# dek226/CSE375-FinalProj-Huffman-Decoding

Measured on AMD Instinct MI355X. Metric: decoded GB/s, higher is better.
Workload: dtype u8

## Files before the change

### cse375-finalproj-huffman-decoding_amd/csrc/gh_tile.hip

```cpp

#ifndef GH_TILE_TB
#define GH_TILE_TB 1024
#endif
constexpr int TILE_TB = GH_TILE_TB;
#ifndef GH_TILE_U
#define GH_TILE_U 3
#endif
constexpr int TILE_U = GH_TILE_U;
constexpr int TILE_U3 = 2;
constexpr int TILE_NS = 4;
constexpr int TILE_SCAP = 20;
constexpr int TILE_MIDG = 2;
constexpr int STAGE_PAD = 16;
#ifndef GH_TILE_LAG
#define GH_TILE_LAG 2
#endif
constexpr int TILE_LAG = GH_TILE_LAG;
constexpr int TILE_SLOTS = 16;
#ifndef GH_TILE_STAMPS
#define GH_TILE_STAMPS 0
#endif
#if GH_TILE_STAMPS
#define TSTAMP(i) (ts[i] = __builtin_amdgcn_s_memtime())
#else
#define TSTAMP(i) ((void)0)
#endif
#ifndef GH_TILE_CSUB
#define GH_TILE_CSUB 0
#endif
#ifndef GH_TILE_CLDS
#define GH_TILE_CLDS 0
#endif
#ifndef GH_TILE_LMAJ
#define GH_TILE_LMAJ 1
#endif
#ifndef GH_TILE_POLLDIV
#define GH_TILE_POLLDIV 1
#endif
#ifndef GH_TILE_DYN
#define GH_TILE_DYN 0
#endif
constexpr int TILE_TAHEAD = 5;
#ifndef GH_TILE_LATEP
#define GH_TILE_LATEP 0
#endif
#ifndef GH_TILE_EPERM
#define GH_TILE_EPERM 0
#endif
#ifndef GH_TILE_HOLD
#define GH_TILE_HOLD 0
#endif
#ifndef GH_TILE_ALRD
#define GH_TILE_ALRD 1
#endif
#ifndef GH_TILE_W2
#define GH_TILE_W2 0
#endif
#ifndef GH_TILE_PF2
#define GH_TILE_PF2 0
#endif
#ifndef GH_TILE_ABLATE
#define GH_TILE_ABLATE 0
#endif
typedef unsigned int tile_v4u __attribute__((ext_vector_type(4)));
__device__ __forceinline__ void tile_st16(uint4* d, const uint4& v) {
  __builtin_nontemporal_store(tile_v4u{v.x, v.y, v.z, v.w}, (tile_v4u*)d);
}

struct TileParams {
  const uint32_t* payload;
  const uint32_t* gaps;
  const uint32_t* lut;
  uint8_t* out;
  unsigned long long* granules;
  unsigned long long* prefix;
  unsigned int* status;
  unsigned long long* total;
  unsigned long long* stats;
  unsigned long long out_cap;
  unsigned long long nseg;
  unsigned int gap_nib0, first_start, ntiles, kbits, lgr, epoch;
  unsigned int lut_bytes;
  unsigned int idle_block;
  unsigned int stage_bytes;
  unsigned int kbits_c;
  unsigned int fb_hi;
  unsigned int* tickets;
  uint4* stamps;
  unsigned long long* tstamps;
};

inline size_t tile_lds_bytes(size_t lut_bytes, size_t stage_bytes) {
  return lut_bytes + TILE_LAG * (TILE_TB / 64) * stage_bytes + TILE_SLOTS * (2 * (TILE_TB / 64) + 1) * 4 +
         TILE_SLOTS * 12 + 4 * (TILE_TB / 64) + 4 * TILE_SLOTS + 32;
}

__device__ __forceinline__ constexpr uint32_t perm_sel(int j) {
  return j == 0 ? 0x03020105u : j == 1 ? 0x03020500u : j == 2 ? 0x03050100u : 0x05020100u;
}

__device__ __forceinline__ void make_ewin(uint4 w, uint32_t w4, int start, uint32_t S, uint32_t (&e)[5]) {
  const uint32_t r = S - (uint32_t)start;
  e[0] = __builtin_amdgcn_alignbit(0u, w.x, r);
  e[1] = __builtin_amdgcn_alignbit(w.x, w.y, r);
  e[2] = __builtin_amdgcn_alignbit(w.y, w.z, r);
  e[3] = __builtin_amdgcn_alignbit(w.z, w.w, r);
  e[4] = __builtin_amdgcn_alignbit(w.w, w4, r);
}

constexpr uint32_t Q_SYMROOM = 0x7FFFu << 8;
constexpr uint32_t Q_LIVE = 128u << 23;
__device__ __forceinline__ uint32_t q_init(bool act, int start) {
  return ((act ? (uint32_t)(127 - start) : 511u) << 23) | Q_SYMROOM | 32u;
}

template <int N>
__device__ __forceinline__ void lds_wait_n(uint32_t& v) {
  static_assert(N >= 0 && N <= 3, "lgkmcnt 0..3");
  if constexpr (GH_TILE_CLDS) return;
  if constexpr (N == 0) asm volatile("s_waitcnt lgkmcnt(0)" : "+v"(v)::"memory");
  else if constexpr (N == 1) asm volatile("s_waitcnt lgkmcnt(1)" : "+v"(v)::"memory");
  else if constexpr (N == 2) asm volatile("s_waitcnt lgkmcnt(2)" : "+v"(v)::"memory");
  else asm volatile("s_waitcnt lgkmcnt(3)" : "+v"(v)::"memory");
}

template <int G, int U, int OW, int MINL, class Mid>
__device__ __forceinline__ int decode_tile_rolling(uint32_t (&e)[U][5], const int (&start)[U], const bool (&act)[U],
                                                   uint32_t (&ow)[U][OW], uint32_t (&cnt)[U], uint32_t amask,
                                                   uint32_t laneoff, Mid&& mid) {
  constexpr int S = 4 * OW;
  constexpr int NG = (S + G - 1) / G;
  constexpr int PLACE = GH_TILE_EPERM ? GH_TILE_EPERM : (G >= 4 ? 2 : 0);
  uint32_t q[U], ent[U];
#if GH_TILE_CLDS
  const __attribute__((address_space(3))) uint8_t* const lds0 = (const __attribute__((address_space(3))) uint8_t*)nullptr;
  auto lut_rd = [&](uint32_t a) -> uint32_t { return *(const __attribute__((address_space(3))) uint32_t*)(lds0 + a); };
#else
  auto lut_rd = [&](uint32_t a) -> uint32_t { return lds_u32_nowait(a); };
#endif
#pragma unroll
  for (int u = 0; u < U; ++u) {
    q[u] = q_init(act[u], start[u]);
    cnt[u] = 0;
#pragma unroll
    for (int k = 0; k < OW; ++k) asm volatile("" : "=v"(ow[u][k]));
  }
#pragma unroll
  for (int u = 0; u < U; ++u) ent[u] = lut_rd((e[u][0] & amask) | laneoff);
  int gdone = NG;
#pragma clang loop unroll(full)
  for (int gi = 0; gi < NG; ++gi) {
    const int CMIN = (gi + 1) * G * MINL;
    uint32_t qmin = 0xFFFFFFFFu;
#pragma clang loop unroll(full)
    for (int j = 0; j < G; ++j) {
      const int pos = gi * G + j;
      if (pos < S) {
        const bool gend = (j == G - 1) || (pos + 1 >= S);
        const bool last = gend && gi + 1 >= NG;
#pragma clang loop unroll(full)
        for (int u = 0; u < U; ++u) {
          if (last) {
            if constexpr (U == 3) {
              if (u == 0) lds_wait_n<2>(ent[u]);
              else if (u == 1) lds_wait_n<1>(ent[u]);
              else lds_wait_n<0>(ent[u]);
            } else if constexpr (U == 2) {
              if (u == 0) lds_wait_n<1>(ent[u]);
              else lds_wait_n<0>(ent[u]);
            } else {
              lds_wait_n<0>(ent[u]);
            }
          } else {
            lds_wait_n<U - 1>(ent[u]);
          }
#if GH_TILE_CSUB
          {
            uint32_t nq;
            const bool br = __builtin_sub_overflow(q[u], ent[u], &nq);
            q[u] = nq;
            cnt[u] = br ? (uint32_t)(pos + 1) : cnt[u];
          }
#else
          asm("v_sub_co_u32 %0, vcc, %0, %2\n\t"
              "v_cndmask_b32_e64 %1, %1, %3, vcc"
              : "+v"(q[u]), "+v"(cnt[u]) : "v"(ent[u]), "i"(pos + 1) : "vcc");
#endif
          ow[u][pos >> 2] = __builtin_amdgcn_perm(ent[u], ow[u][pos >> 2], perm_sel(pos & 3));
          if (PLACE == 1) asm volatile("" : "+v"(ow[u][pos >> 2]));
          if (!gend) {
            const uint32_t x = __builtin_amdgcn_alignbit(e[u][0], e[u][1], q[u]);
            ent[u] = lut_rd((x & amask) | laneoff);
          } else {
            e[u][0] = __builtin_amdgcn_alignbit(e[u][0], e[u][1], q[u]);
            if (CMIN + 32 < 157) e[u][1] = __builtin_amdgcn_alignbit(e[u][1], e[u][2], q[u]);
            if (CMIN + 64 < 157) e[u][2] = __builtin_amdgcn_alignbit(e[u][2], e[u][3], q[u]);
            if (CMIN + 96 < 157) e[u][3] = __builtin_amdgcn_alignbit(e[u][3], e[u][4], q[u]);
            if (CMIN + 128 < 157) e[u][4] = __builtin_amdgcn_alignbit(e[u][4], 0u, q[u]);
            q[u] = (q[u] & 0xFFFFFF00u) | 32u;
            qmin = min(qmin, q[u]);
            if (!last) ent[u] = lut_rd((e[u][0] & amask) | laneoff);
          }
        }
      }
    }
    if (PLACE == 2) {
#pragma unroll
      for (int u = 0; u < U; ++u) {
        const int w0 = (gi * G) >> 2, w1 = min(OW - 1, (gi * G + G - 1) >> 2);
#pragma unroll
        for (int wi = w0; wi <= w1; ++wi) asm volatile("" : "+v"(ow[u][wi]));
      }
    }
    if (gi == TILE_MIDG) mid();
    if (gi >= TILE_MIDG && gi + 1 < NG && !__any(qmin < Q_LIVE)) {
#pragma unroll
      for (int u = 0; u < U; ++u) lds_wait_n<0>(ent[u]);
      gdone = gi + 1;
      break;
    }
  }
  return gdone;
}

template <int OFF = 0>
__device__ __forceinline__ void lds_st32(uint32_t a, uint32_t v) {
  asm volatile("ds_write_b32 %0, %1 offset:%2" ::"v"(a), "v"(v), "i"(OFF) : "memory");
}
__device__ __forceinline__ uint32_t lds_ld_u32(uint32_t a) {
  uint32_t v;
  asm volatile("ds_read_b32 %0, %1\n\ts_waitcnt lgkmcnt(0)" : "=v"(v) : "v"(a) : "memory");
  return v;
}
__device__ __forceinline__ void lds_st_u32(uint32_t a, uint32_t v) {
  asm volatile("ds_write_b32 %0, %1\n\ts_waitcnt lgkmcnt(0)" ::"v"(a), "v"(v) : "memory");
}
__device__ __forceinline__ void lds_st32_m(uint32_t a, uint32_t v, int m) {
  switch (m) {
    case 1: lds_st32<4>(a, v); break;
    case 2: lds_st32<8>(a, v); break;
    case 3: lds_st32<12>(a, v); break;
    case 4: lds_st32<16>(a, v); break;
    case 5: lds_st32<20>(a, v); break;
    case 6: lds_st32<24>(a, v); break;
    case 7: lds_st32<28>(a, v); break;
    case 8: lds_st32<32>(a, v); break;
    case 9: lds_st32<36>(a, v); break;
    case 10: lds_st32<40>(a, v); break;
    case 11: lds_st32<44>(a, v); break;
    default: lds_st32<0>(a + 4u * (uint32_t)m, v); break;
  }
}
template <int U, int OW>
__device__ __forceinline__ void stage_wave(const uint32_t (&ow)[U][OW], const uint32_t (&n)[U], const uint32_t (&o)[U],
                                           int mmax) {
  uint32_t base[U], sh[U];
#pragma unroll
  for (int u = 0; u < U; ++u) {
    const uint32_t ap = ((o[u] - 1u) & 3u) + 1u;
    base[u] = o[u] - ap;
    sh[u] = 4u - ap;
  }
  auto dw = [&](int u, int m) { return __builtin_amdgcn_alignbyte(m < OW ? ow[u][m] : 0u, ow[u][m - 1], sh[u]); };
  if constexpr (GH_TILE_W2) {
#pragma unroll
    for (int m = OW; m >= 1; m -= 2) {
      if (m - 1 >= 1) {
        if (m <= mmax) {
#pragma unroll
          for (int u = 0; u < U; ++u)
            asm volatile("ds_write2_b32 %0, %1, %2 offset0:%3 offset1:%4" ::"v"(base[u]), "v"(dw(u, m)),
                         "v"(dw(u, m - 1)), "i"(m), "i"(m - 1) : "memory");
        } else if (m - 1 <= mmax) {
#pragma unroll
          for (int u = 0; u < U; ++u) lds_st32_m(base[u], dw(u, m - 1), m - 1);
        }
      } else if (m <= mmax) {
#pragma unroll
        for (int u = 0; u < U; ++u) lds_st32_m(base[u], dw(u, m), m);
      }
    }
  } else {
#pragma unroll
    for (int m = OW; m >= 1; --m) {
      if (m > mmax) continue;
#pragma unroll
      for (int u = 0; u < U; ++u) lds_st32_m(base[u], dw(u, m), m);
    }
  }
  uint32_t rd[U];
#pragma unroll
  for (int u = 0; u < U; ++u) rd[u] = lds_u32_nowait(base[u]);
  lds_wait(rd);
#pragma unroll
  for (int u = 0; u < U; ++u) {
    const uint32_t ap = o[u] - base[u];
    if (n[u] && ap < 4u) {
      const uint32_t ab = 8u * ap;
      lds_st32(base[u], (rd[u] & ((1u << ab) - 1u)) | (ow[u][0] << ab));
    }
  }
}

constexpr uint32_t OOB_OFF = 0x80000000u;
template <int NS, bool PIN = true>
__device__ __forceinline__ void copy_out_piece(uint8_t* out, uint32_t stg, unsigned long long goff, uint32_t n,
                                               int lane, tile_v4u (&v)[NS], uint32_t& b, uint32_t c0 = 0) {
  goff = rfl_u64(goff);
  n = (uint32_t)__builtin_amdgcn_readfirstlane((int)n);
  const uint32_t lb = (uint32_t)(goff & 15);
  const __amdgpu_buffer_rsrc_t rs = __builtin_amdgcn_make_buffer_rsrc(out + (goff - lb), 0, 0x7FFFFFF0, 0x00020000);
  const uint32_t src = (stg + 16u - ((GH_TILE_ABLATE & 128) ? 0u : lb)) & ((GH_TILE_ABLATE & 256) ? ~3u : ~0u);
  const uint32_t cf = lb ? 1u : 0u;
  const uint32_t ce = n ? (lb + n) >> 4 : 0u;
  uint32_t off[NS];
#pragma unroll
  for (int i = 0; i < NS; ++i) {
    const uint32_t c = c0 + cf + (uint32_t)lane + 64u * (uint32_t)i;
    off[i] = c < ce ? 16u * c : OOB_OFF;
  }
  const uint32_t nh = (lb && n) ? min(16u, lb + n) - lb : 0u;
  const uint32_t tl = (lb + n) & 15u;
  const uint32_t nt = (n && tl && (ce > 0 || !lb)) ? tl : 0u;
  const uint32_t t = (uint32_t)lane;
  uint32_t k = OOB_OFF;
  if (c0 == 0u && !(GH_TILE_ABLATE & 64)) {
    if (t < nh) k = lb + t;
    else if (t < nh + nt) k = 16u * ce + (t - nh);
  }
  if constexpr (GH_TILE_ALRD) {
    constexpr int CG = NS % 2 == 0 ? 2 : 1;
    const uint32_t sh = (16u - lb) & 15u, r = sh & 3u, m = lb ? sh >> 2 : 4u;
    if constexpr (GH_TILE_ALRD == 2) {
      tile_v4u P[NS + 1];
#pragma unroll
      for (int i = 0; i <= NS; ++i) {
        const uint32_t c = c0 + cf + (uint32_t)lane + 64u * (uint32_t)i;
        const uint32_t a = stg + 16u * (c < ce + 1u ? c : cf);
        asm volatile("ds_read_b128 %0, %1" : "=v"(P[i]) : "v"(a) : "memory");
      }
      if (PIN) asm volatile("ds_read_u8 %0, %1" : "+v"(b) : "v"(src + (k == OOB_OFF ? 0u : k)) : "memory");
      else asm volatile("ds_read_u8 %0, %1" : "=v"(b) : "v"(src + (k == OOB_OFF ? 0u : k)) : "memory");
      asm volatile("s_waitcnt lgkmcnt(0)" ::: "memory");
#pragma unroll
      for (int i = 0; i <= NS; ++i) asm volatile("" : "+v"(P[i]));
#pragma unroll
      for (int i = 0; i < NS; ++i) {
        tile_v4u Q;
#pragma unroll
        for (int d = 0; d < 4; ++d) {
          const int nx = __builtin_amdgcn_update_dpp(0, (int)P[i + 1][d], 0x134, 0xf, 0xf, false);
          Q[d] = (uint32_t)__builtin_amdgcn_update_dpp(nx, (int)P[i][d], 0x130, 0xf, 0xf, false);
        }
        auto W = [&](int q) -> uint32_t { return q < 4 ? P[i][q] : Q[q - 4]; };
        switch (m) {
          case 0:
            for (int d = 0; d < 4; ++d) v[i][d] = __builtin_amdgcn_alignbyte(W(d + 1), W(d), r);
            break;
          case 1:
            for (int d = 0; d < 4; ++d) v[i][d] = __builtin_amdgcn_alignbyte(W(d + 2), W(d + 1), r);
            break;
          case 2:
            for (int d = 0; d < 4; ++d) v[i][d] = __builtin_amdgcn_alignbyte(W(d + 3), W(d + 2), r);
            break;
          case 3:
            for (int d = 0; d < 4; ++d) v[i][d] = __builtin_amdgcn_alignbyte(W(d + 4), W(d + 3), r);
            break;
          default:
            v[i] = Q;
            break;
        }
        __builtin_amdgcn_raw_buffer_store_b128(v[i], rs, (int)off[i], 0, 2);
      }
      if (PIN) asm volatile("" : "+v"(b));
      __builtin_amdgcn_raw_buffer_store_b8((uint8_t)b, rs, (int)k, 0, 2);
      return;
    }
#pragma unroll
    for (int g0 = 0; g0 < NS; g0 += CG) {
      tile_v4u pq[CG][2];
#pragma unroll
      for (int j = 0; j < CG; ++j) {
        const int i = g0 + j;
        const uint32_t c = c0 + cf + (uint32_t)lane + 64u * (uint32_t)i;
        const uint32_t a = stg + 16u * (c < ce ? c : cf);
        asm volatile("ds_read_b128 %0, %1" : "=v"(pq[j][0]) : "v"(a) : "memory");
        asm volatile("ds_read_b128 %0, %1 offset:16" : "=v"(pq[j][1]) : "v"(a) : "memory");
      }
      if (g0 + CG >= NS) {
        if (PIN) asm volatile("ds_read_u8 %0, %1" : "+v"(b) : "v"(src + (k == OOB_OFF ? 0u : k)) : "memory");
        else asm volatile("ds_read_u8 %0, %1" : "=v"(b) : "v"(src + (k == OOB_OFF ? 0u : k)) : "memory");
      }
      asm volatile("s_waitcnt lgkmcnt(0)" ::: "memory");
#pragma unroll
      for (int j = 0; j < CG; ++j) asm volatile("" : "+v"(pq[j][0]), "+v"(pq[j][1]));
      auto shift = [&](auto mc) {
        constexpr int M = decltype(mc)::value;
#pragma unroll
        for (int j = 0; j < CG; ++j) {
          if constexpr (M == 4) {
            v[g0 + j] = pq[j][1];
          } else {
            auto W = [&](int q) -> uint32_t { return q < 4 ? pq[j][0][q] : pq[j][1][q - 4]; };
#pragma unroll
            for (int d = 0; d < 4; ++d) v[g0 + j][d] = __builtin_amdgcn_alignbyte(W(M + d + 1), W(M + d), r);
          }
        }
      };
      switch (m) {
        case 0: shift(std::integral_constant<int, 0>{}); break;
        case 1: shift(std::integral_constant<int, 1>{}); break;
        case 2: shift(std::integral_constant<int, 2>{}); break;
        case 3: shift(std::integral_constant<int, 3>{}); break;
        default: shift(std::integral_constant<int, 4>{}); break;
      }
#pragma unroll
      for (int j = 0; j < CG; ++j) __builtin_amdgcn_raw_buffer_store_b128(v[g0 + j], rs, (int)off[g0 + j], 0, 2);
    }
    if (PIN) asm volatile("" : "+v"(b));
    __builtin_amdgcn_raw_buffer_store_b8((uint8_t)b, rs, (int)k, 0, 2);
    return;
  }
#pragma unroll
  for (int i = 0; i < NS; ++i) {
    const uint32_t c = c0 + cf + (uint32_t)lane + 64u * (uint32_t)i;
    if (PIN) asm volatile("ds_read_b128 %0, %1" : "+v"(v[i]) : "v"(src + 16u * (c < ce ? c : cf)) : "memory");
    else asm volatile("ds_read_b128 %0, %1" : "=v"(v[i]) : "v"(src + 16u * (c < ce ? c : cf)) : "memory");
  }
  if (PIN) asm volatile("ds_read_u8 %0, %1" : "+v"(b) : "v"(src + (k == OOB_OFF ? 0u : k)) : "memory");
  else asm volatile("ds_read_u8 %0, %1" : "=v"(b) : "v"(src + (k == OOB_OFF ? 0u : k)) : "memory");
  asm volatile("s_waitcnt lgkmcnt(0)" : "+v"(b)::"memory");
#pragma unroll
  for (int i = 0; i < NS; ++i) asm volatile("" : "+v"(v[i]));
#pragma unroll
  for (int i = 0; i < NS; ++i) __builtin_amdgcn_raw_buffer_store_b128(v[i], rs, (int)off[i], 0, 2);
  __builtin_amdgcn_raw_buffer_store_b8((uint8_t)b, rs, (int)k, 0, 2);
}

template <int OW>
__device__ __forceinline__ void store_direct(uint8_t* out, unsigned long long cap, unsigned long long o,
                                             const uint32_t (&ow)[OW], uint32_t n) {
#pragma unroll
  for (int i = 0; i < 4 * OW; ++i)
    if ((uint32_t)i < n && o + (uint32_t)i < cap) out[o + (uint32_t)i] = (uint8_t)(ow[i >> 2] >> (8 * (i & 3)));
}

__device__ __forceinline__ bool granule_ok(const TileParams& p, unsigned long long v, uint32_t flag) {
  return (uint32_t)(v >> 40) == p.epoch && (uint32_t)((v >> 38) & 3u) == flag;
}

__device__ __forceinline__ unsigned long long poll_granule(const TileParams& p, unsigned long long* g,
                                                           uint32_t flag) {
  unsigned long long t0 = 0;
  for (uint32_t spins = 1;; ++spins) {
    const unsigned long long v = __hip_atomic_load(g, __ATOMIC_RELAXED, __HIP_MEMORY_SCOPE_AGENT);
    if (granule_ok(p, v, flag)) return v;
    if ((spins & 63u) == 0u) {
      if (__hip_atomic_load(p.status, __ATOMIC_RELAXED, __HIP_MEMORY_SCOPE_AGENT) & GH_ST_TIMEOUT) return 0;
      const unsigned long long t = wall_clock64();
      if (t0 == 0) {
        t0 = t;
      } else if (t - t0 > 400000000ull) {
        atomicOr(p.status, (unsigned)GH_ST_TIMEOUT);
        return 0;
      }
    }
    __builtin_amdgcn_s_sleep(2);
  }
}

constexpr int LEAD_A = 4;
template <int TB>
__device__ __forceinline__ void tile_round_leader(const TileParams& p, uint32_t D, uint32_t* s_lead, int tid,
                                                  int lane, int wid) {
  const uint32_t A = (D + TB - 1) / TB;
  const uint32_t nr = (p.ntiles + D - 1) / D;
  unsigned long long R = 0;
  for (uint32_t r = 0; r < nr; ++r) {
    const uint32_t t0 = r * D, n = min(D, p.ntiles - t0);
    uint32_t v[LEAD_A], sum = 0;
#pragma unroll
    for (int i = 0; i < LEAD_A; ++i) {
      const uint32_t j = (uint32_t)tid * A + (uint32_t)i;
      v[i] = 0;
      if ((uint32_t)i < A && j < n) {
        unsigned long long g = __hip_atomic_load(&p.granules[t0 + j], __ATOMIC_RELAXED, __HIP_MEMORY_SCOPE_AGENT);
        if (!granule_ok(p, g, 1)) {
          atomicAdd(p.stats + 1, 1ull);
          g = poll_granule(p, &p.granules[t0 + j], 1);
        }
        v[i] = (uint32_t)(g & GRAN_VMASK);
      }
      sum += v[i];
    }
    const uint32_t incl = wave_incl_scan(sum);
    if (lane == 63) s_lead[wid] = incl;
    __syncthreads();
    unsigned long long before = 0, total = 0;
#pragma unroll
    for (int q = 0; q < TB / 64; ++q) {
      const uint32_t x = s_lead[q];
      before += (q < wid) ? x : 0u;
      total += x;
    }
    unsigned long long run = R + before + incl - sum;
#pragma unroll
    for (int i = 0; i < LEAD_A; ++i) {
      const uint32_t j = (uint32_t)tid * A + (uint32_t)i;
      if ((uint32_t)i < A && j < n)
        __hip_atomic_store(&p.prefix[t0 + j], granule(p.epoch, 2, run), __ATOMIC_RELAXED, __HIP_MEMORY_SCOPE_AGENT);
      run += v[i];
    }
    R += total;
#if GH_TILE_STAMPS
    if (tid == 0) p.tstamps[2 * p.ntiles + r] = __builtin_amdgcn_s_memrealtime();
#endif
    __syncthreads();
  }
}

template <int TB>
__device__ __forceinline__ void tile_frontier_leader(const TileParams& p, uint32_t* s_w, int tid, int lane, int wid) {
  constexpr int NW = TB / 64;
  uint32_t F = 0;
  unsigned long long R = 0, t0 = 0;
  uint32_t* const s_first = s_w;
  uint32_t* const s_sum = s_w + 2 * NW;
  for (uint32_t pass = 0; F < p.ntiles; ++pass) {
    const uint32_t t = F + (uint32_t)tid, pb = (pass & 1u) * NW;
    bool in = false;
    uint32_t v = 0;
    if (t < p.ntiles) {
      const unsigned long long g = __hip_atomic_load(&p.granules[t], __ATOMIC_RELAXED, __HIP_MEMORY_SCOPE_AGENT);
      in = granule_ok(p, g, 1);
      v = (uint32_t)(g & GRAN_VMASK);
    }
    const unsigned long long out = __ballot(!in);
    if (lane == 0) s_first[pb + wid] = out ? (uint32_t)__builtin_ctzll(out) : 64u;
    __syncthreads();
    uint32_t m = (uint32_t)TB;
#pragma unroll
    for (int q = NW - 1; q >= 0; --q) {
      const uint32_t f = s_first[pb + q];
      m = f < 64u ? 64u * (uint32_t)q + f : m;
    }
    const uint32_t vv = (uint32_t)tid < m ? v : 0u;
    const uint32_t incl = wave_incl_scan(vv);
    if (lane == 63) s_sum[pb + wid] = incl;
    __syncthreads();
    unsigned long long before = 0, total = 0;
#pragma unroll
    for (int q = 0; q < NW; ++q) {
      const uint32_t x = s_sum[pb + q];
      before += (q < wid) ? x : 0u;
      total += x;
    }
    if ((uint32_t)tid < m) {
      __hip_atomic_store(&p.prefix[t], granule(p.epoch, 2, R + before + incl - vv), __ATOMIC_RELAXED,
                         __HIP_MEMORY_SCOPE_AGENT);
#if GH_TILE_STAMPS
      p.tstamps[2 * p.ntiles + t] = __builtin_amdgcn_s_memrealtime();
#endif
    }
    R += total;
    F += m;
    if (m == 0u) {
      if (tid == 0) atomicAdd(p.stats + 1, 1ull);
      if ((pass & 63u) == 0u) {
        if (__hip_atomic_load(p.status, __ATOMIC_RELAXED, __HIP_MEMORY_SCOPE_AGENT) & GH_ST_TIMEOUT) return;
        const unsigned long long tw = wall_clock64();
        if (t0 == 0) {
          t0 = tw;
        } else if (tw - t0 > 400000000ull) {
          if (tid == 0) atomicOr(p.status, (unsigned)GH_ST_TIMEOUT);
          return;
        }
      }
      __builtin_amdgcn_s_sleep(2);
    } else {
      t0 = 0;
    }
  }
}

template <int TB, int U, int GRP, int OW, int MINL>
__global__ __launch_bounds__(TB) __attribute__((amdgpu_waves_per_eu(4, 4))) void gh_tile_kernel(const TileParams p) {
  static_assert(4 * OW >= (128 + MINL - 1) / MINL, "OW words hold every codeword a segment can start");
  static_assert(U <= TILE_U, "shapes of at most TILE_U segments per lane");
  constexpr int NW = TB / 64;
  extern __shared__ __attribute__((aligned(16))) uint8_t smem[];
  const uint32_t stage_lds = p.lut_bytes;
  uint32_t* s_tot = (uint32_t*)(smem + p.lut_bytes + TILE_LAG * NW * p.stage_bytes);
  uint32_t* s_off = s_tot + TILE_SLOTS * NW;
  uint32_t* s_cnt = s_off + TILE_SLOTS * NW;
  unsigned long long* s_pfx = (unsigned long long*)(s_cnt + TILE_SLOTS);
  uint32_t* s_ptile = (uint32_t*)(s_pfx + TILE_SLOTS);
  uint32_t* s_lead = s_ptile + TILE_SLOTS;
  uint32_t* s_ring = s_lead + NW;
  const uint32_t cnt_lds = (uint32_t)((uint8_t*)s_cnt - smem);
  const uint32_t ptile_lds = (uint32_t)((uint8_t*)s_ptile - smem);
  const uint32_t ring_lds = (uint32_t)((uint8_t*)s_ring - smem);

  const int tid = threadIdx.x, lane = tid & 63, wid = tid >> 6;
#if GH_TILE_STAMPS
  unsigned long long* const lring = p.tstamps + 3ull * p.ntiles + 64 + 4ull * (p.epoch & 1023u);
  if (blockIdx.x == 0 && tid == 0) {
    lring[0] = __builtin_amdgcn_s_memtime();
    lring[1] = __builtin_amdgcn_s_memrealtime();
  }
#endif
  const uint32_t D = gridDim.x - 1 - (p.idle_block < gridDim.x ? 1u : 0u);
  if (blockIdx.x == 0) {
    if constexpr (GH_TILE_DYN) {
      if (tid == 0) p.tickets[2u * ((p.epoch + 1u) & 1u)] = 0u;
      tile_frontier_leader<TB>(p, (uint32_t*)smem, tid, lane, wid);
    } else {
      tile_round_leader<TB>(p, D, s_lead, tid, lane, wid);
    }
#if GH_TILE_STAMPS
    if (tid == 0) {
      lring[2] = __builtin_amdgcn_s_memtime();
      lring[3] = __builtin_amdgcn_s_memrealtime();
    }
#endif
    return;
  }
  if (blockIdx.x == p.idle_block) return;
#if GH_TILE_STAMPS
  unsigned long long* const wring = p.tstamps + 3ull * p.ntiles + 64 + 4ull * 1024 + 4ull * blockIdx.x;
  if (tid == 0) {
    wring[0] = __builtin_amdgcn_s_memtime();
    wring[1] = __builtin_amdgcn_s_memrealtime();
  }
#endif
  {
    const uint32_t nd = p.lut_bytes >> 2;
    uint32_t* sl = (uint32_t*)smem;
    for (uint32_t i = tid; i < nd; i += TB) sl[i] = p.lut[i >> p.lgr];
    if (tid < TILE_SLOTS) {
      s_cnt[tid] = 0;
      s_ptile[tid] = 0xFFFFFFFFu;
    }
    if (GH_TILE_DYN && tid <= TILE_TAHEAD) {
      const uint32_t b0 = blockIdx.x - 1 - (blockIdx.x > p.idle_block ? 1u : 0u);
      const uint32_t tt = b0 + (uint32_t)tid * D;
      s_ring[tid] = tt < p.ntiles ? tt : 0xFFFFFFFFu;
    }
  }
  const uint32_t S = 30u - p.kbits - p.lgr;
  const uint32_t amask = (((1u << p.kbits) - 1u) << (2u + p.lgr)) & ((GH_TILE_ABLATE & 16) ? ~(1u << (2u + p.lgr)) : ~0u);
  const uint32_t laneoff = ((uint32_t)lane & ((1u << p.lgr) - 1u)) << 2;
  check_lds_base(smem, p.status);

  const uint32_t G = D, b = blockIdx.x - 1 - (blockIdx.x > p.idle_block ? 1u : 0u);
  const uint32_t nseg = (uint32_t)p.nseg;
  constexpr uint32_t NONE = 0xFFFFFFFFu;
  __syncthreads();
  const uint32_t last_tile_k = GH_TILE_DYN ? p.ntiles + 2u * TILE_SLOTS
                               : b < p.ntiles ? (p.ntiles - 1 - b) / G : NONE;
  uint32_t cur = b, nxt = b + G;
  const uint32_t dyn_base = (uint32_t)(TILE_TAHEAD + 1) * D;
  uint32_t tk = 0;
  bool tk_live = GH_TILE_DYN && dyn_base < p.ntiles;
  unsigned int* const tctr = GH_TILE_DYN ? p.tickets + 2u * (p.epoch & 1u) : nullptr;
  constexpr uint32_t CSTR = GH_TILE_LMAJ ? 1u : 64u;
  const uint32_t lseg = (uint32_t)(wid * 64 * U) + (uint32_t)lane * (GH_TILE_LMAJ ? (uint32_t)U : 1u);
  constexpr int NSET = GH_TILE_PF2 ? 2 : 1;
  static_assert(!(GH_TILE_PF2 && (GH_TILE_DYN || GH_TILE_HOLD)), "PF2: static schedule, no hold");
  uint4 wset[NSET][U];
  uint32_t w4set[NSET][U], gwset[NSET][U];
  auto load = [&](auto SS, uint32_t t) {
    constexpr int SI = decltype(SS)::value;
    uint4 (&w)[U] = wset[SI];
    uint32_t (&w4)[U] = w4set[SI];
    uint32_t (&gw)[U] = gwset[SI];
    const uint32_t seg0 = min(t, p.ntiles - 1) * (uint32_t)(U * TB) + lseg;
    if constexpr (GH_TILE_LMAJ) {
      const uint32_t sb = min(seg0, nseg - 1);
#pragma unroll
      for (int u = 0; u < U; ++u) w[u] = *(const uint4*)(p.payload + 4ull * (sb + (uint32_t)u));
      w4[U - 1] = p.payload[4ull * (sb + (uint32_t)U)];
#pragma unroll
      for (int u = 0; u < U; ++u) {
        const uint32_t sc = sb + (uint32_t)u;
        gw[u] = p.gaps[(p.gap_nib0 + (sc ? sc - 1u : 0u)) >> 3];
      }
    } else {
#pragma unroll
      for (int u = 0; u < U; ++u) {
        const uint32_t sc = min(seg0 + (uint32_t)(64 * u), nseg - 1);
        w[u] = *(const uint4*)(p.payload + 4ull * sc);
        w4[u] = p.payload[4ull * sc + 4];
        gw[u] = p.gaps[(p.gap_nib0 + (sc ? sc - 1u : 0u)) >> 3];
      }
    }
  };
  const __amdgpu_buffer_rsrc_t rs_out = __builtin_amdgcn_make_buffer_rsrc(p.out, 0, 0x7FFFFFF0, 0x00020000);
  auto ticket_op = [&]() {
    if constexpr (GH_TILE_DYN) {
      if (wid == 0 && tk_live) {
        if (lane == 0) tk = atomicAdd(tctr, 1u);
      } else {
        __builtin_amdgcn_raw_buffer_store_b8((uint8_t)0, rs_out, (int)(OOB_OFF + 64u), 0, 2);
      }
    }
  };
  auto junk_stores = [&]() {
    const __amdgpu_buffer_rsrc_t rs = rs_out;
#pragma unroll
    for (int i = 0; i < TILE_NS; ++i)
      __builtin_amdgcn_raw_buffer_store_b128(tile_v4u{0, 0, 0, 0}, rs, (int)(OOB_OFF + 16u * (uint32_t)i), 0, 2);
    __builtin_amdgcn_raw_buffer_store_b8((uint8_t)0, rs, (int)OOB_OFF, 0, 2);
  };
  load(std::integral_constant<int, 0>{}, cur);
  ticket_op();
  junk_stores();
  if constexpr (GH_TILE_PF2) {
    (void)__hip_atomic_load(&p.prefix[0], __ATOMIC_RELAXED, __HIP_MEMORY_SCOPE_AGENT);
    (void)__hip_atomic_load(&p.prefix[0], __ATOMIC_RELAXED, __HIP_MEMORY_SCOPE_AGENT);
    load(std::integral_constant<int, NSET - 1>{}, nxt);
    junk_stores();
  }
  if (cur >= p.ntiles) cur = NONE;
  uint32_t th[TILE_LAG];
#pragma unroll
  for (int i = 0; i < TILE_LAG; ++i) th[i] = NONE;
  uint32_t owp[U][OW], cntp[U], bposp[U], wtp = 0, prevt = NONE;
  int gdp = 1;
#pragma unroll
  for (int u = 0; u < U; ++u) {
    cntp[u] = 0;
    bposp[u] = 0;
#pragma unroll
    for (int k2 = 0; k2 < OW; ++k2) asm volatile("" : "=v"(owp[u][k2]));
  }
  uint32_t rank = 0;
  const uint32_t region0 = stage_lds + (uint32_t)wid * p.stage_bytes;
  const uint32_t piece_cap = p.stage_bytes - (uint32_t)(STAGE_PAD + 4 * OW + 4);
#if GH_TILE_STAMPS
  unsigned long long ts[9];
#endif
  auto body = [&](auto SS, uint32_t k) -> bool {
    constexpr int SI = decltype(SS)::value;
    uint4 (&w)[U] = wset[SI];
    uint32_t (&w4)[U] = w4set[SI];
    uint32_t (&gw)[U] = gwset[SI];
    TSTAMP(0);
    const bool have_cur = cur < p.ntiles;
    const uint32_t t2 = th[TILE_LAG - 1];
    const bool have2 = t2 < p.ntiles;
    bool pending = have_cur || (GH_TILE_HOLD && prevt < p.ntiles);
#pragma unroll
    for (int i = 0; i < TILE_LAG; ++i) pending |= th[i] < p.ntiles;
    if (!pending) return false;
    if (last_tile_k != NONE && k > last_tile_k + TILE_LAG + 2) {
      if (lane == 0) atomicOr(p.status, (unsigned)GH_ST_TIMEOUT);
      return false;
    }
    const uint32_t slot = k % TILE_SLOTS, slot2 = (k + TILE_SLOTS - TILE_LAG - GH_TILE_HOLD) % TILE_SLOTS;
    const uint32_t slotp = (k + TILE_SLOTS - 1) % TILE_SLOTS;
    const uint32_t buf = k % TILE_LAG;
    if (rank >= 3) __builtin_amdgcn_s_setprio(3);
    else if (rank == 2) __builtin_amdgcn_s_setprio(2);
    else if (rank == 1) __builtin_amdgcn_s_setprio(1);
    else __builtin_amdgcn_s_setprio(0);
    unsigned long long* const pf2 = &p.prefix[have2 ? t2 : 0u];
    unsigned long long gp0 = 0, gp = 0, gpl = 0;
    if (!(GH_TILE_ABLATE & 4)) gp0 = __hip_atomic_load(pf2, __ATOMIC_RELAXED, __HIP_MEMORY_SCOPE_AGENT);
    auto mid = [&]() {
      if (!(GH_TILE_ABLATE & 4)) gp = __hip_atomic_load(pf2, __ATOMIC_RELAXED, __HIP_MEMORY_SCOPE_AGENT);
    };
    const uint32_t seg0 = cur * (uint32_t)(U * TB) + lseg;
    uint32_t ow[U][OW], cnt[U];
    int gdone;
    {
      int start[U];
      bool act[U];
      uint32_t e[U][5];
#pragma unroll
      for (int u = 0; u < U; ++u) {
        const uint32_t seg = seg0 + (uint32_t)u * CSTR;
        act[u] = have_cur && seg < nseg;
        start[u] = seg == 0 ? (int)p.first_start : (int)gap_nib(gw[u], p.gap_nib0 + seg - 1u);
        make_ewin(w[u], (GH_TILE_LMAJ && u + 1 < U) ? w[u + 1 < U ? u + 1 : u].x : w4[u], start[u], S, e[u]);
      }
      TSTAMP(1);
      if (GH_TILE_ABLATE & 1) {
#pragma unroll
        for (int u = 0; u < U; ++u) {
          cnt[u] = act[u] ? 16u : 0u;
#pragma unroll
          for (int k2 = 0; k2 < OW; ++k2) ow[u][k2] = e[u][k2 % 5];
        }
        mid();
        gdone = (16 + GRP - 1) / GRP;
      } else {
        gdone = decode_tile_rolling<GRP, U, OW, MINL>(e, start, act, ow, cnt, amask, laneoff, mid);
      }
    }
    if constexpr (GH_TILE_DYN) {
      if (wid == 0) {
        uint32_t tpost = NONE;
        if (lane == 0 && tk_live) tpost = dyn_base + tk < p.ntiles ? dyn_base + tk : NONE;
        tpost = (uint32_t)__builtin_amdgcn_readfirstlane((int)tpost);
        tk_live = tk_live && tpost != NONE;
        if (lane == 0) lds_st_u32(ring_lds + 4u * ((k + 1u + TILE_TAHEAD) % TILE_SLOTS), tpost);
      }
      nxt = lds_ld_u32(ring_lds + 4u * ((k + 1u) % TILE_SLOTS));
      nxt = (uint32_t)__builtin_amdgcn_readfirstlane((int)nxt);
    }
    if (GH_TILE_LATEP && !(GH_TILE_ABLATE & 4)) gpl = __hip_atomic_load(pf2, __ATOMIC_RELAXED, __HIP_MEMORY_SCOPE_AGENT);
    load(SS, GH_TILE_PF2 ? nxt + G : nxt);
    ticket_op();
    TSTAMP(2);
    uint32_t bpos[U], wave_tot = 0;
    if constexpr (GH_TILE_LMAJ) {
      uint32_t sl = 0;
#pragma unroll
      for (int u = 0; u < U; ++u) sl += cnt[u];
      const uint32_t incl = wave_incl_scan(sl);
      uint32_t run = incl - sl;
#pragma unroll
      for (int u = 0; u < U; ++u) {
        bpos[u] = run;
        run += cnt[u];
      }
      wave_tot = (uint32_t)__builtin_amdgcn_readlane((int)incl, 63);
    } else {
#pragma unroll
      for (int u = 0; u < U; ++u) bpos[u] = wave_incl_scan(cnt[u]);
#pragma unroll
      for (int u = 0; u < U; ++u) {
        const uint32_t ct = (uint32_t)__builtin_amdgcn_readlane((int)bpos[u], 63);
        bpos[u] += wave_tot - cnt[u];
        wave_tot += ct;
      }
    }
    uint32_t tile_total = 0;
    if (have_cur) {
      uint32_t old = 0;
      if (lane == 0) {
        s_tot[slot * NW + wid] = wave_tot;
        asm volatile("ds_add_rtn_u32 %0, %1, %2\n\ts_waitcnt lgkmcnt(0)" : "=v"(old) : "v"(cnt_lds + 4u * slot), "v"(1u)
                     : "memory");
      }
      const uint32_t arr = (uint32_t)__builtin_amdgcn_readfirstlane((int)old);
      rank = (4u * arr) / NW;
      if (arr == NW - 1) {
        const uint32_t x = lane < NW ? s_tot[slot * NW + lane] : 0u;
        const uint32_t xi = wave_incl_scan(x);
        if (lane < NW) s_off[slot * NW + lane] = xi - x;
        tile_total = (uint32_t)__builtin_amdgcn_readlane((int)xi, NW - 1);
        if (lane == 0) {
          s_cnt[slot] = 0;
          asm volatile("s_waitcnt lgkmcnt(0)" ::: "memory");
          __hip_atomic_store(&p.granules[cur], granule(p.epoch, 1, tile_total), __ATOMIC_RELAXED,
                             __HIP_MEMORY_SCOPE_AGENT);
#if GH_TILE_STAMPS
          p.tstamps[cur] = __builtin_amdgcn_s_memrealtime();
#endif
        }
      }
    }
    TSTAMP(3);
    unsigned long long goff = 0;
    uint32_t n2 = 0;
    if (have2 && (GH_TILE_ABLATE & 4)) {
      goff = ((unsigned long long)t2 * (U * TB * 16) + (uint32_t)wid * (U * 64 * 16)) % (p.out_cap - (U * TB * 32));
      n2 = s_tot[slot2 * NW + wid];
    } else if (have2) {
      unsigned long long g = rfl_u64(gp0);
      bool polled = false, got = true;
      (void)polled;
      if (!granule_ok(p, g, 2)) g = rfl_u64(gp);
      if (GH_TILE_LATEP && !granule_ok(p, g, 2)) g = rfl_u64(gpl);
      {
        if (!granule_ok(p, g, 2)) {
          polled = true;
          if (wid == 0 && lane == 0) atomicAdd(p.stats, 1ull);
          unsigned long long t0w = 0;
          unsigned long long pv = __hip_atomic_load(pf2, __ATOMIC_RELAXED, __HIP_MEMORY_SCOPE_AGENT);
          for (uint32_t spins = 1;; ++spins) {
            bool found = false;
            if (lds_ld_u32(ptile_lds + 4u * slot2) == t2) {
              asm volatile("" ::: "memory");
              g = s_pfx[slot2];
              found = true;
            } else {
              g = rfl_u64(pv);
              if (granule_ok(p, g, 2)) {
                if (lane == 0) {
                  s_pfx[slot2] = g;
                  asm volatile("s_waitcnt lgkmcnt(0)" ::: "memory");
                  lds_st_u32(ptile_lds + 4u * slot2, t2);
                }
                found = true;
              } else if (GH_TILE_POLLDIV <= 1 || ((spins + (uint32_t)wid) % GH_TILE_POLLDIV) == 0u) {
                pv = __hip_atomic_load(pf2, __ATOMIC_RELAXED, __HIP_MEMORY_SCOPE_AGENT);
              }
            }
            if (found) break;
            if ((spins & 63u) == 0u) {
              if (__hip_atomic_load(p.status, __ATOMIC_RELAXED, __HIP_MEMORY_SCOPE_AGENT) & GH_ST_TIMEOUT) break;
              const unsigned long long t = wall_clock64();
              if (t0w == 0) {
                t0w = t;
              } else if (t - t0w > 400000000ull) {
                if (lane == 0) atomicOr(p.status, (unsigned)GH_ST_TIMEOUT);
                break;
              }
            }
            __builtin_amdgcn_s_sleep(1);
          }
          got = granule_ok(p, g, 2);
        }
      }
      asm volatile("" ::: "memory");
      goff = (g & GRAN_VMASK) + s_off[slot2 * NW + wid];
      if (GH_TILE_ABLATE & 32) goff &= ~15ull;
      n2 = s_tot[slot2 * NW + wid];
      if (wid == NW - 1 && t2 == p.ntiles - 1 && got && lane == 0) *p.total = goff + n2;
#if GH_TILE_STAMPS
      if (wid == 0 && lane == 0) p.tstamps[p.ntiles + t2] = __builtin_amdgcn_s_memrealtime() | ((unsigned long long)polled << 63);
#endif
      n2 = (!got || goff >= p.out_cap) ? 0u : (uint32_t)min<unsigned long long>(n2, p.out_cap - goff);
    }
    TSTAMP(4);
    if (!(GH_TILE_ABLATE & 8)) {
      tile_v4u cv[TILE_NS];
      uint32_t cb;
      copy_out_piece<TILE_NS, false>(p.out, region0 + buf * NW * p.stage_bytes, goff, n2, lane, cv, cb);
    }
    TSTAMP(5);
    const uint32_t st_t = GH_TILE_HOLD ? prevt : cur;
    const bool have_st = st_t < p.ntiles;
    const uint32_t st_tot = GH_TILE_HOLD ? wtp : wave_tot;
    const uint32_t st_slot = GH_TILE_HOLD ? slotp : slot;
    const bool staged = have_st && st_tot <= piece_cap;
    auto stage_or_store = [&](const uint32_t (&sow)[U][OW], const uint32_t (&scnt)[U], const uint32_t (&sbpos)[U],
                              int sgd) {
      if (have_st && !staged) {
        unsigned long long goffc = 0;
        bool got = true;
        if (lane == 0) {
          unsigned long long g = __hip_atomic_load(&p.prefix[st_t], __ATOMIC_RELAXED, __HIP_MEMORY_SCOPE_AGENT);
          if (!granule_ok(p, g, 2)) g = poll_granule(p, &p.prefix[st_t], 2);
          got = granule_ok(p, g, 2);
          asm volatile("" ::: "memory");
          goffc = (g & GRAN_VMASK) + s_off[st_slot * NW + wid];
          if (wid == NW - 1 && st_t == p.ntiles - 1 && got) *p.total = goffc + st_tot;
        }
        goffc = rfl_u64(goffc);
        if (__builtin_amdgcn_readfirstlane(got ? 1 : 0)) {
#pragma unroll
          for (int u = 0; u < U; ++u) store_direct(p.out, p.out_cap, goffc + sbpos[u], sow[u], scnt[u]);
        }
        __builtin_amdgcn_s_waitcnt(0x0F70);
      } else if (have_st && !(GH_TILE_ABLATE & 2)) {
        const uint32_t sbase = region0 + buf * NW * p.stage_bytes + STAGE_PAD;
        uint32_t o[U];
#pragma unroll
        for (int u = 0; u < U; ++u) o[u] = sbase + sbpos[u];
        stage_wave<U, OW>(sow, scnt, o, min(OW, (GRP * sgd + 3) >> 2));
      }
    };
    if constexpr (GH_TILE_HOLD) {
      stage_or_store(owp, cntp, bposp, gdp);
#pragma unroll
      for (int u = 0; u < U; ++u) {
        cntp[u] = cnt[u];
        bposp[u] = bpos[u];
#pragma unroll
        for (int k2 = 0; k2 < OW; ++k2) owp[u][k2] = ow[u][k2];
      }
      wtp = wave_tot;
      gdp = gdone;
    } else {
      stage_or_store(ow, cnt, bpos, gdone);
    }
    TSTAMP(6);
#if GH_TILE_STAMPS
    TSTAMP(7);
    TSTAMP(8);
    if (lane == 0 && (wid == 0 || wid == NW / 2) && k < 128) {
      uint4* st = p.stamps + (((unsigned long long)blockIdx.x * 2 + (wid ? 1 : 0)) * 128 + k) * 2;
      st[0] = make_uint4((uint32_t)(ts[1] - ts[0]), (uint32_t)(ts[2] - ts[1]), (uint32_t)(ts[3] - ts[2]),
                         (uint32_t)(ts[4] - ts[3]));
      st[1] = make_uint4((uint32_t)(ts[5] - ts[4]), (uint32_t)(ts[6] - ts[5]), (uint32_t)(ts[7] - ts[6]),
                         (uint32_t)(ts[8] - ts[7]));
    }
#endif
#pragma unroll
    for (int i = TILE_LAG - 1; i > 0; --i) th[i] = th[i - 1];
    th[0] = staged ? st_t : NONE;
    if constexpr (GH_TILE_HOLD) prevt = have_cur ? cur : NONE;
    cur = nxt < p.ntiles ? nxt : NONE;
    if constexpr (!GH_TILE_DYN) nxt += G;
    return true;
  };
  for (uint32_t k = 0;; k += NSET) {
    if (!body(std::integral_constant<int, 0>{}, k)) break;
    if constexpr (NSET == 2) {
      if (!body(std::integral_constant<int, NSET - 1>{}, k + 1)) break;
    }
  }
#if GH_TILE_STAMPS
  if (tid == 0) {
    wring[2] = __builtin_amdgcn_s_memtime();
    wring[3] = __builtin_amdgcn_s_memrealtime();
  }
#endif
}
```

Baseline: 2351.

## Skip borrow tracking in never-borrow prefix and pair-pack output bytes

Within the provable never-borrow prefix of each tile decode, the subtract-with-carry plus conditional move becomes a plain subtract, and the live-check reduction is skipped until that prefix ends. Output symbol bytes are packed in pairs and then quads with fewer v_perm ops instead of one perm per symbol, and partial words are flushed on early exit. An idle-wave early exit at the mid point is added when there is no tile. This shortens the per-symbol ALU chain, but correctness relies on static maxlen bounds and the new flush logic.

```diff
diff --git a/cse375-finalproj-huffman-decoding_amd/csrc/gh_tile.hip b/cse375-finalproj-huffman-decoding_amd/csrc/gh_tile.hip
--- a/cse375-finalproj-huffman-decoding_amd/csrc/gh_tile.hip
+++ b/cse375-finalproj-huffman-decoding_amd/csrc/gh_tile.hip
@@ -25,9 +25,6 @@
 #else
 #define TSTAMP(i) ((void)0)
 #endif
-#ifndef GH_TILE_CSUB
-#define GH_TILE_CSUB 0
-#endif
 #ifndef GH_TILE_CLDS
 #define GH_TILE_CLDS 0
 #endif
@@ -43,9 +40,6 @@
 constexpr int TILE_TAHEAD = 5;
 #ifndef GH_TILE_LATEP
 #define GH_TILE_LATEP 0
-#endif
-#ifndef GH_TILE_EPERM
-#define GH_TILE_EPERM 0
 #endif
 #ifndef GH_TILE_HOLD
 #define GH_TILE_HOLD 0
@@ -95,9 +89,9 @@
          TILE_SLOTS * 12 + 4 * (TILE_TB / 64) + 4 * TILE_SLOTS + 32;
 }
 
-__device__ __forceinline__ constexpr uint32_t perm_sel(int j) {
-  return j == 0 ? 0x03020105u : j == 1 ? 0x03020500u : j == 2 ? 0x03050100u : 0x05020100u;
-}
+constexpr uint32_t PERM_PAIR = 0x07060501u;
+constexpr uint32_t PERM_QUAD = 0x05040100u;
+constexpr uint32_t PERM_THIRD = 0x07050100u;
 
 __device__ __forceinline__ void make_ewin(uint4 w, uint32_t w4, int start, uint32_t S, uint32_t (&e)[5]) {
   const uint32_t r = S - (uint32_t)start;
@@ -127,11 +121,18 @@
 template <int G, int U, int OW, int MINL, class Mid>
 __device__ __forceinline__ int decode_tile_rolling(uint32_t (&e)[U][5], const int (&start)[U], const bool (&act)[U],
                                                    uint32_t (&ow)[U][OW], uint32_t (&cnt)[U], uint32_t amask,
-                                                   uint32_t laneoff, Mid&& mid) {
+                                                   uint32_t laneoff, bool have_tile, Mid&& mid) {
   constexpr int S = 4 * OW;
   constexpr int NG = (S + G - 1) / G;
-  constexpr int PLACE = GH_TILE_EPERM ? GH_TILE_EPERM : (G >= 4 ? 2 : 0);
-  uint32_t q[U], ent[U];
+  static_assert(G >= 2 && G <= 4, "G = min(4, 32 / maxlen) with maxlen <= 12");
+  constexpr int LMAX = G >= 4 ? 8 : G == 3 ? 10 : 12;
+  static_assert(G * LMAX <= 32 && (G == 4 || (G + 1) * LMAX > 32), "LMAX is the longest maxlen with 32 / maxlen == G");
+  constexpr int NB = 112 / LMAX;
+  static_assert(15 + NB * LMAX <= 127 && NB < S, "the never-borrow prefix");
+  constexpr int GLIVE = NB / G;
+  static_assert(GLIVE >= TILE_MIDG && GLIVE < NG, "mid() runs before any exit");
+  constexpr bool PLACE = G >= 4;
+  uint32_t q[U], ent[U], hold[U], pair[U];
 #if GH_TILE_CLDS
   const __attribute__((address_space(3))) uint8_t* const lds0 = (const __attribute__((address_space(3))) uint8_t*)nullptr;
   auto lut_rd = [&](uint32_t a) -> uint32_t { return *(const __attribute__((address_space(3))) uint32_t*)(lds0 + a); };
@@ -174,20 +175,20 @@
           } else {
             lds_wait_n<U - 1>(ent[u]);
           }
-#if GH_TILE_CSUB
-          {
-            uint32_t nq;
-            const bool br = __builtin_sub_overflow(q[u], ent[u], &nq);
-            q[u] = nq;
-            cnt[u] = br ? (uint32_t)(pos + 1) : cnt[u];
+          if (pos < NB) {
+            q[u] -= ent[u];
+          } else {
+            asm("v_sub_co_u32 %0, vcc, %0, %2\n\t"
+                "v_cndmask_b32_e64 %1, %1, %3, vcc"
+                : "+v"(q[u]), "+v"(cnt[u]) : "v"(ent[u]), "i"(pos + 1) : "vcc");
           }
-#else
-          asm("v_sub_co_u32 %0, vcc, %0, %2\n\t"
-              "v_cndmask_b32_e64 %1, %1, %3, vcc"
-              : "+v"(q[u]), "+v"(cnt[u]) : "v"(ent[u]), "i"(pos + 1) : "vcc");
-#endif
-          ow[u][pos >> 2] = __builtin_amdgcn_perm(ent[u], ow[u][pos >> 2], perm_sel(pos & 3));
-          if (PLACE == 1) asm volatile("" : "+v"(ow[u][pos >> 2]));
+          if ((pos & 1) == 0) {
+            hold[u] = ent[u];
+          } else if ((pos & 3) == 1) {
+            pair[u] = __builtin_amdgcn_perm(ent[u], hold[u], PERM_PAIR);
+          } else {
+            ow[u][pos >> 2] = __builtin_amdgcn_perm(__builtin_amdgcn_perm(ent[u], hold[u], PERM_PAIR), pair[u], PERM_QUAD);
+          }
           if (!gend) {
             const uint32_t x = __builtin_amdgcn_alignbit(e[u][0], e[u][1], q[u]);
             ent[u] = lut_rd((x & amask) | laneoff);
@@ -198,13 +199,13 @@
             if (CMIN + 96 < 157) e[u][3] = __builtin_amdgcn_alignbit(e[u][3], e[u][4], q[u]);
             if (CMIN + 128 < 157) e[u][4] = __builtin_amdgcn_alignbit(e[u][4], 0u, q[u]);
             q[u] = (q[u] & 0xFFFFFF00u) | 32u;
-            qmin = min(qmin, q[u]);
+            if (gi >= GLIVE) qmin = min(qmin, q[u]);
             if (!last) ent[u] = lut_rd((e[u][0] & amask) | laneoff);
           }
         }
       }
     }
-    if (PLACE == 2) {
+    if (PLACE) {
 #pragma unroll
       for (int u = 0; u < U; ++u) {
         const int w0 = (gi * G) >> 2, w1 = min(OW - 1, (gi * G + G - 1) >> 2);
@@ -213,9 +214,16 @@
       }
     }
     if (gi == TILE_MIDG) mid();
-    if (gi >= TILE_MIDG && gi + 1 < NG && !__any(qmin < Q_LIVE)) {
+    if (gi + 1 < NG && (gi >= GLIVE ? !__any(qmin < Q_LIVE) : (gi == TILE_MIDG && !have_tile))) {
 #pragma unroll
       for (int u = 0; u < U; ++u) lds_wait_n<0>(ent[u]);
+      const int pe = gi * G + G - 1;
+#pragma unroll
+      for (int u = 0; u < U; ++u) {
+        if ((pe & 3) == 0) ow[u][pe >> 2] = hold[u] >> 8;
+        else if ((pe & 3) == 1) ow[u][pe >> 2] = pair[u];
+        else if ((pe & 3) == 2) ow[u][pe >> 2] = __builtin_amdgcn_perm(hold[u], pair[u], PERM_THIRD);
+      }
       gdone = gi + 1;
       break;
     }
@@ -795,7 +803,7 @@
         mid();
         gdone = (16 + GRP - 1) / GRP;
       } else {
-        gdone = decode_tile_rolling<GRP, U, OW, MINL>(e, start, act, ow, cnt, amask, laneoff, mid);
+        gdone = decode_tile_rolling<GRP, U, OW, MINL>(e, start, act, ow, cnt, amask, laneoff, have_cur, mid);
       }
     }
     if constexpr (GH_TILE_DYN) {
```

New measurement: 2392, median of 6. +1.7%, better.
